# sherholz/mitsuba-path-guiding

Measured on AMD Instinct MI355X. Metric: Mpaths/sec + equal-spp RMSE vs CPU ref, ajar-door scene at 1/2/4/8 GPUs, higher is better.
Workload: dtype f32; 1 GPU; C3 ajar_door 1280x720, guided SD-tree, 5 training iterations (1..16 spp) + 1024 spp render; scene=ajar_door, triangles=58864, width=1280, height=720, spp=1024, parallelism=tile-shard x1, no exchange (one rank)

## Files before the change

### mitsuba-path-guiding_amd/csrc/pg_kernels.h

```cpp
#pragma once
#include <hip/hip_runtime.h>
#include <stdint.h>

#include "pg_layout.h"

struct SceneDev {
    const float4 *nodes;
    const float4 *tris;
    const float4 *wnodes;
    const float4 *wtris;
    const float4 *tshade;
    const uint8_t *tclass;
    const GMat *mats;
    const GEmitter *ems;
    const float4 *emtri;
    const float *emcdf;
    const GEnv *env;
    uint32_t top_nodes;
    uint32_t num_em_boxes;
    float em_absmax;
    float em_box[PG_EMBOX_MAX][6];
    uint32_t num_blockers;
    float absmax;
    uint32_t *blk_counts;
// ... 116 lines not shown
inline uint32_t pg_camera_bound(bool banded, uint32_t npix, uint32_t nlayers) {
    uint32_t b = 0;
    for (uint32_t s = 0; s < 64; ++s) {
        const uint32_t c = pg_camera_count(banded, npix, nlayers, s);
        b = c > b ? c : b;
    }
    return b;
}

void pg_launch_camera(hipStream_t s, const GParams &g, const PathDev &p, const uint32_t *local_pixels,
                      uint32_t pix_begin, uint32_t npix, uint32_t nlayers, uint32_t sample_base, Queue q, bool banded);
void pg_launch_camera_rays(hipStream_t s, const GParams &g, const uint32_t *pixels, const uint32_t *samples, uint32_t n,
                           float *o_tmin, float *d_tmax);
void pg_launch_trace(hipStream_t s, const GParams &g, const SceneDev &sc, const PathDev &p, Queue q, uint32_t max_shard,
                     const Queue *class_queues, bool first_bounce);
void pg_launch_camera_trace(hipStream_t s, const GParams &g, const SceneDev &sc, const PathDev &p,
                            const uint32_t *local_pixels, uint32_t pix_begin, uint32_t npix, uint32_t nlayers,
                            uint32_t sample_base, const Queue *class_queues);
void pg_launch_camera_queue(hipStream_t s, uint32_t npix, uint32_t nlayers, Queue q);
void pg_launch_shade_class(hipStream_t s, int cls, const GParams &g, const SceneDev &sc, const SDDev &sd,
                           const PathDev &p, Queue in, uint32_t max_shard, Queue out, Queue shadow, Queue probe);
void pg_launch_shade_all(hipStream_t s, const GParams &g, const SceneDev &sc, const SDDev &sd, const PathDev &p,
                         const Queue *class_queues, const uint32_t *max_shard, Queue out, Queue shq, Queue probe);
void pg_launch_rays(hipStream_t s, const GParams &g, const SceneDev &sc, const PathDev &p, Queue q, uint32_t max_shard,
                    const Queue *class_queues, Queue shq, uint32_t max_shadow_shard, Queue probe);
void pg_launch_shadow(hipStream_t s, const GParams &g, const SceneDev &sc, const PathDev &p, Queue q, uint32_t max_shard);
void pg_launch_probe(hipStream_t s, const SceneDev &sc, const PathDev &p, Queue probe, uint32_t max_shard,
                     const Queue *class_queues);
void pg_launch_tail(hipStream_t s, const GParams &g, const SceneDev &sc, const SDDev &sd, const PathDev &p, Queue q,
                    uint32_t max_shard, unsigned long long *stats);
void pg_launch_ray_sort(hipStream_t s, Queue q, uint32_t max_shard, uint32_t *sorted_items, uint32_t *hist,
                        uint32_t bins = PG_RAY_SORT_BINS);
void pg_launch_film(hipStream_t s, const GParams &g, const SceneDev &sc, const PathDev &p, const uint32_t *local_pixels,
                    uint32_t pix_begin, uint32_t npix, uint32_t nlayers, float4 *film_rgbw, float4 *film_sumsq,
                    float4 *aov_albedo = nullptr, float4 *aov_normal = nullptr);
struct FilmFilter {
    float radius, scale;
    int32_t border;
// ... 63 lines not shown
```

### mitsuba-path-guiding_amd/csrc/pg_kernels.hip

```cpp
#include <algorithm>
#include <cstdlib>

#include "pg_trace.h"

#ifndef SHADE_LDS_MATS
#define SHADE_LDS_MATS 0
#endif

template <bool LENS>
__global__ __launch_bounds__(256) void k_camera(GParams g, PathDev p, const uint32_t *__restrict__ local_pixels,
                                                uint32_t pix_begin, uint32_t npix, uint32_t nlayers,
                                                uint32_t sample_base, Queue q, bool banded) {
    uint32_t slot = blockIdx.x * blockDim.x + threadIdx.x;
    const uint32_t n = npix * nlayers;
    if (slot < PG_QSHARDS) q.counts[slot] = pg_camera_count(banded, npix, nlayers, slot);
    if (slot >= n) return;
    uint32_t layer = slot / npix, lp = slot - layer * npix;
    uint32_t pix = local_pixels[pix_begin + lp];
    uint32_t sample = sample_base + layer;
    f3 o, wd;
    float tmin, tmax;
    cameraRay<LENS>(g, pix, rngKey(pix, g.seed), sample, o, wd, tmin, tmax);
    stS(pathRayO(p, slot), f4(o, tmin));
    stS(pathRayD(p, slot), f4(wd, tmax));
// ... 122 lines not shown
            }
            cls = hitClass(sc, h, tri, doomed, hr);
            stS(&p.hit[slot], hr);
        }
        classAppend(cls, slot, cqs, s);
    }
}

template <bool ENV, bool CAM>
__global__ __launch_bounds__(TRACE_BLOCK) void k_trace(GParams g, SceneDev sc, PathDev p, Queue q, ClassQueues cqs,
                                                       float4 *first) {
    __shared__ uint32_t stack[LDS_STACK * TRACE_BLOCK];
    traceRows<ENV, CAM>(g, sc, p, q, cqs, first, blockIdx.x, gridDim.x, threadStack(stack, p.stack_ovf));
}

struct CameraChunk {
    const uint32_t *local_pixels;
    uint32_t pix_begin, npix, nlayers, sample_base;
};
template <bool ENV, bool LENS>
__device__ __forceinline__ void cameraRows(const GParams &g, const SceneDev &sc, const PathDev &p, const CameraChunk &cam,
                                           const ClassQueues &cqs, float4 *first, uint32_t bid, uint32_t nblk,
                                           const TStack &stk) {
    const uint32_t s = bid & (PG_QSHARDS - 1);
    const uint32_t n = pg_camera_shard_count(cam.npix * cam.nlayers, s);
    for (uint32_t base = (bid / PG_QSHARDS) * TRACE_BLOCK; base < n; base += nblk / PG_QSHARDS * TRACE_BLOCK) {
        const uint32_t i = base + threadIdx.x;
        int cls = -1;
        uint32_t slot = 0;
        if (i < n) {
            slot = pg_camera_slot(s, i);
            f3 o, wd;
            float tmin, tmax;
            {
                const uint32_t layer = slot / cam.npix, lp = slot - layer * cam.npix;
                const uint32_t pix = cam.local_pixels[cam.pix_begin + lp];
                const uint32_t sample = cam.sample_base + layer;
                cameraRay<LENS>(g, pix, rngKey(pix, g.seed), sample, o, wd, tmin, tmax);
                stS(pathRayD(p, slot), f4(wd, tmax));
                stS(&p.rad[slot], make_float4(0.f, 0.f, 0.f, 0.f));
                stS(pathInfo(p, slot), make_uint4(pix, sample, kCameraWord, 0u));
            }
            const float far = tmax;
            uint32_t tri = 0xFFFFFFFFu;
            float u = 0, v = 0;
            const bool h = traverse<false>(sc.nodes, sc.tris, o, wd, tmin, tmax, tri, u, v, stk);
            float4 hr = make_float4(h ? tmax : 0.0f, __uint_as_float(h ? tri : 0xFFFFFFFFu), u, v);
            if (first) first[slot] = hr;
            if (ENV && !h) {
                const f3 e = envEscapeRadiance(g, sc, p, slot, wd, kCameraWord, far);
                hr = make_float4(e.x, hr.y, e.y, e.z);
            }
            cls = hitClass(sc, h, tri, false, hr);
            stS(&p.hit[slot], hr);
        }
        classAppend(cls, slot, cqs, s);
    }
}
template <bool ENV, bool LENS>
__global__ __launch_bounds__(TRACE_BLOCK) __attribute__((amdgpu_waves_per_eu(LENS ? 4 : ENV ? 5 : 6))) void k_camera_trace(GParams g, SceneDev sc, PathDev p, CameraChunk cam,
                                                              ClassQueues cqs, float4 *first) {
    __shared__ uint32_t stack[LDS_STACK * TRACE_BLOCK];
    cameraRows<ENV, LENS>(g, sc, p, cam, cqs, first, blockIdx.x, gridDim.x, threadStack(stack, p.stack_ovf));
}

__device__ __forceinline__ float shadowTmin(float4 o) {
    return kEpsilon * fmaxf(fmaxf(fabsf(o.x), fabsf(o.y)), fabsf(o.z));
}

template <class T>
__device__ __forceinline__ void waveKeyedAdd(T *base, uint32_t key, T v, bool valid);
__device__ __forceinline__ bool blockerRowCounted(uint32_t row) { return row % PG_BLOCKER_SAMPLE == 0; }
__device__ __forceinline__ void shadowAdd(const PathDev &p, uint32_t slot) {
    float4 c = ldS(&p.sh_c[slot]);
    float4 L = ldS(&p.rad[slot]);
    stS(&p.rad[slot], make_float4(L.x + c.x, L.y + c.y, L.z + c.z, L.w));
    uint32_t vi = __float_as_uint(c.w);
    if (vi != 0xFFFFFFFFu) {
// ... 202 lines not shown
extern "C" int pg_debug_watch_read(float *out, uint32_t max, uint32_t *n) {
    uint32_t w[3];
    if (hipDeviceSynchronize() != hipSuccess) return -1;
    if (hipMemcpyFromSymbol(w, HIP_SYMBOL(pgWatch), sizeof(w)) != hipSuccess) return -1;
    *n = w[2] < PG_WATCH_MAX ? w[2] : PG_WATCH_MAX;
    const uint32_t k = *n < max ? *n : max;
    return hipMemcpyFromSymbol(out, HIP_SYMBOL(pgWatchLog), (size_t)k * PG_WATCH_F * 4) == hipSuccess ? 0 : -1;
}
#define WSET(i, v) (wr[i] = (float)(v))
#define WSET3(i, v) (wr[i] = (v).x, wr[(i) + 1] = (v).y, wr[(i) + 2] = (v).z)
#else
#define WSET(i, v) ((void)0)
#define WSET3(i, v) ((void)0)
#endif

template <int MODEL, bool CAN_GUIDE, bool ENV, bool TEX = false, bool DELTA = false>
__device__ __forceinline__ void shadeOne(const GParams &g, const SceneDev &sc, const SDDev &sd, const PathDev &p,
                                         uint32_t slot, const GMat *mats, bool wantKey, bool &alive, bool &shadow,
                                         bool &probe, uint32_t &rkey, uint32_t &blocked) {
    bool dirtyL = false;
    f3 L = mk1(0.f);
    const bool cull = !PG_WATCH && g.path_cull;
#if PG_WATCH
    float wr[PG_WATCH_F];
    for (int i = 0; i < PG_WATCH_F; ++i) wr[i] = -1.0f;
    bool watched = false;
#endif
    do {
        const uint4 pi = ldS(pathInfo(p, slot));
        const uint32_t pix = pi.x, sample = pi.y;
#if PG_WATCH
        watched = pix == pgWatch[0] && sample == pgWatch[1];
#endif
        const float4 rd4 = ldS(pathRayD(p, slot));
        float4 hv = ldS(&p.hit[slot]);
        uint32_t depth = pi.z & 0xFFFFu, flags = pi.z >> 16, nv = pi.w;
        float4 T4 = depth == 1 ? make_float4(1.f, 1.f, 1.f, 1.f) : ldS(pathThr(p, slot));
        f3 T = xyz(T4);
        bool haveL = depth == 1;
        auto loadL = [&]() {
            if (!haveL) {
                L = xyz(ldS(&p.rad[slot]));
                haveL = true;
            }
        };
        if (PG_WATCH) loadL();
        float eta = T4.w;
        uint32_t tri = __float_as_uint(hv.y);
        if (tri == 0xFFFFFFFFu) break;
        const uint32_t key = rngKey(pix, g.seed);
        f3 rd = xyz(rd4);
        Hit h;
        fetchHit(sc, tri, hv.z, hv.w, rd, h);
        WSET(0, depth);
        WSET(1, __float_as_uint(sc.tshade[(size_t)PG_TRI_SHADE_STRIDE * tri + 2].w));
        WSET3(2, h.p);
        f3 Le = mk1(0.f);
        if (h.emitter >= 0 && dot(h.shN, -rd) > 0) {
            const GEmitter &em = sc.ems[h.emitter];
            Le = mk(em.radiance[0], em.radiance[1], em.radiance[2]);
        }
        if (depth > 1) {
            if (h.emitter >= 0) {
                const float prevPdf = rd4.w;
                float lumPdf = 0.0f;
                if (g.use_nee && !(flags & PF_PREV_DELTA)) {
// ... 194 lines not shown
                             (D - 1 >= (uint32_t)g.rr_depth && rrNext >= fminf(maxc(Tn) * etaN * etaN, 0.95f));
                }
                if (!ENV && doomed && g.doom_probe) {
                    const float po[3] = {h.p.x, h.p.y, h.p.z}, pd[3] = {wo.x, wo.y, wo.z};
                    probe = pg_ray_misses_boxes(sc.em_box, sc.num_em_boxes, sc.em_absmax, po, pd, tmin);
                }
                stS(pathRayO(p, slot), f4(h.p, doomed ? -tmin : tmin));
                stS(pathRayD(p, slot), f4(wo, woPdf));
                if (probe) {
                    stS(&p.hit[slot], make_float4(0.0f, __uint_as_float(0xFFFFFFFFu), 0.0f, 0.0f));
                } else {
                    stS(pathThr(p, slot), f4(Tn, etaN));
                    flags = (flags & ~(PF_EMITTED_QUERY | PF_PREV_DELTA | PF_PREV_FRONT)) |
                        ((bs.type & EDelta) ? PF_PREV_DELTA : 0u) | (doomed ? PF_DOOMED : 0u) |
                        (pg_prev_front(wo.x, wo.y, wo.z, refN.x, refN.y, refN.z) ? PF_PREV_FRONT : 0u);
                    stPinfoZW(pathInfo(p, slot), (depth + 1) | (flags << 16), nv);
                    alive = true;
                    if (wantKey) rkey = rayOrderKey(sd, h.p, wo);
                }
            }
        }
        if (shadow) {
            if (!alive && !probe) stS(pathRayO(p, slot), f4(h.p, 0.0f));
            stS(&p.sh_d[slot], f4(neeD, neeDist * (1 - kShadowEpsilon)));
            stS(&p.sh_c[slot], f4(neeC, __uint_as_float(vtxIndex)));
        }
        if (!alive && nv != pi.w) stPinfoZW(pathInfo(p, slot), pi.z, nv);
    } while (false);
    if (dirtyL) stS(&p.rad[slot], f4(L, 0.0f));
#if PG_WATCH
    if (watched) {
        wr[28] = alive ? 1.0f : 0.0f;
        wr[29] = shadow ? 1.0f : 0.0f;
        const uint32_t k = atomicAdd(&pgWatch[2], 1u);
        if (k < PG_WATCH_MAX)
            for (int i = 0; i < PG_WATCH_F; ++i) pgWatchLog[k * PG_WATCH_F + i] = wr[i];
    }
#endif
}

template <int MODEL, bool CAN_GUIDE, bool ENV, bool TEX = false, bool DELTA = false>
__device__ __forceinline__ void shadeBlock(const GParams &g, const SceneDev &sc, const SDDev &sd, const PathDev &p,
                                           const Queue &in, const Queue &out, const Queue &shq, const Queue &pq,
                                           uint32_t bid) {
    const uint32_t s = bid & (PG_QSHARDS - 1);
    const uint32_t n = in.counts[s];
    {
    const uint32_t base = (bid / PG_QSHARDS) * SHADE_BLOCK;
    if (base >= n) return;
    const uint32_t i = base + threadIdx.x;
    bool alive = false, shadow = false, probe = false;
    uint32_t slot = 0, rkey = 0, blocked = 0;
    if (i < n) slot = in.items[(size_t)s * in.stride + i];
    __shared__ float4 smat[(SHADE_LDS_MATS > 0 ? SHADE_LDS_MATS : 1) * (sizeof(GMat) / 16)];
    const bool ldsMats = SHADE_LDS_MATS > 0 && g.num_materials <= SHADE_LDS_MATS;
    if (ldsMats) {
        const float4 *src = reinterpret_cast<const float4 *>(sc.mats);
        for (uint32_t k = threadIdx.x; k < g.num_materials * (uint32_t)(sizeof(GMat) / 16); k += SHADE_BLOCK) smat[k] = src[k];
        __syncthreads();
    }
    if (i < n)
        shadeOne<MODEL, CAN_GUIDE, ENV, TEX, DELTA>(g, sc, sd, p, slot, ldsMats ? reinterpret_cast<const GMat *>(smat) : sc.mats,
                                        out.keys != nullptr, alive, shadow, probe, rkey, blocked);
    if (out.keys)
        waveAppendKey(alive, slot, (uint16_t)rkey, out.items + (size_t)s * out.stride, out.keys + (size_t)s * out.stride,
                      out.counts + s);
    else
        waveAppend(alive, slot, out.items + (size_t)s * out.stride, out.counts + s);
    waveAppend(shadow, slot, shq.items + (size_t)s * shq.stride, shq.counts + s);
    if (!ENV && sc.num_blockers) {
        const unsigned long long m = __ballot(blocked != 0);
        if (m) {
            if ((threadIdx.x & 63) == 0) atomicAdd(shq.dropped + s, (uint32_t)__popcll(m));
            if (sc.blk_counts && blockerRowCounted(bid / PG_QSHARDS)) {
                waveKeyedAdd<uint32_t>(sc.blk_counts, blocked - 1u, 1u, blocked != 0);
                if ((threadIdx.x & 63) == 0) atomicAdd(sc.blk_total, (uint32_t)__popcll(m));
            }
        }
// ... 2 lines not shown
    }
}

template <int MODEL, bool CAN_GUIDE, bool ENV, bool TEX = false, bool DELTA = false>
__global__ __launch_bounds__(SHADE_BLOCK) void k_shade(GParams g, SceneDev sc, SDDev sd, PathDev p, Queue in,
                                                       Queue out, Queue shq, Queue pq) {
    shadeBlock<MODEL, CAN_GUIDE, ENV, TEX, DELTA>(g, sc, sd, p, in, out, shq, pq, blockIdx.x);
}

struct ShadeRanges {
    uint32_t end[PG_NUM_CLASSES];
};
#ifndef PG_SHADE_WAVES
#define PG_SHADE_WAVES 4
#endif
template <bool TEX, bool DELTA = false>
__global__ __launch_bounds__(SHADE_BLOCK) __attribute__((amdgpu_waves_per_eu(PG_SHADE_WAVES))) void k_shade_all(
    GParams g, SceneDev sc, SDDev sd, PathDev p, ClassQueues in, Queue out, Queue shq, Queue pq, ShadeRanges r) {
    static_assert(PG_NUM_CLASSES == 7, "class ranges");
    const uint32_t b = blockIdx.x;
    if (b < r.end[0]) shadeBlock<PG_BSDF_DIFFUSE, true, false, false, DELTA>(g, sc, sd, p, in.q[0], out, shq, pq, b);
    else if (b < r.end[1]) shadeBlock<PG_BSDF_ROUGHCONDUCTOR, true, false, false, DELTA>(g, sc, sd, p, in.q[1], out, shq, pq, b - r.end[0]);
    else if (b < r.end[2]) shadeBlock<PG_BSDF_ROUGHDIELECTRIC, true, false, false, DELTA>(g, sc, sd, p, in.q[2], out, shq, pq, b - r.end[1]);
    else if (b < r.end[3]) shadeBlock<PG_BSDF_PLASTIC, false, false, false, DELTA>(g, sc, sd, p, in.q[3], out, shq, pq, b - r.end[2]);
    else if (b < r.end[4]) shadeBlock<PG_BSDF_ROUGHPLASTIC, true, false, false, DELTA>(g, sc, sd, p, in.q[4], out, shq, pq, b - r.end[3]);
    else if (!TEX || b < r.end[5]) shadeBlock<-1, false, false, false, DELTA>(g, sc, sd, p, in.q[5], out, shq, pq, b - r.end[4]);
    else if constexpr (TEX)
        shadeBlock<PG_MODELS_TEXTURED, true, false, true, DELTA>(g, sc, sd, p, in.q[6], out, shq, pq, b - r.end[5]);
}

#define RSORT_TILE 4096
template <uint32_t BINS>
__global__ __launch_bounds__(256) void k_rsort_hist(Queue q, uint32_t *hist) {
    __shared__ uint32_t h[BINS];
    const uint32_t s = blockIdx.x & (PG_QSHARDS - 1), tile = blockIdx.x / PG_QSHARDS;
    const uint32_t n = q.counts[s], b0 = tile * RSORT_TILE;
    if (b0 >= n) return;
    for (uint32_t k = threadIdx.x; k < BINS; k += 256) h[k] = 0;
    __syncthreads();
    const uint16_t *keys = q.keys + (size_t)s * q.stride;
    const uint32_t e = min(n, b0 + RSORT_TILE);
    for (uint32_t i = b0 + threadIdx.x; i < e; i += 256) atomicAdd(&h[keys[i]], 1u);
    __syncthreads();
// ... 772 lines not shown
                     const Queue *class_queues, bool first_bounce) {
    if (!max_shard) return;
    ClassQueues cq;
    for (int c = 0; c < PG_CLASS_ROWS; ++c) cq.q[c] = class_queues[c];
    const dim3 grid = shardGrid(max_shard, TRACE_BLOCK, TRACE_MAX_BLOCKS / PG_QSHARDS);
    float4 *first = first_bounce ? p.aov : nullptr;
    if (first_bounce) {
        if (sc.env) hipLaunchKernelGGL((k_trace<true, true>), grid, dim3(TRACE_BLOCK), 0, s, g, sc, p, q, cq, first);
        else hipLaunchKernelGGL((k_trace<false, true>), grid, dim3(TRACE_BLOCK), 0, s, g, sc, p, q, cq, first);
    } else {
        if (sc.env) hipLaunchKernelGGL((k_trace<true, false>), grid, dim3(TRACE_BLOCK), 0, s, g, sc, p, q, cq, first);
        else hipLaunchKernelGGL((k_trace<false, false>), grid, dim3(TRACE_BLOCK), 0, s, g, sc, p, q, cq, first);
    }
}
void pg_launch_camera_trace(hipStream_t s, const GParams &g, const SceneDev &sc, const PathDev &p,
                            const uint32_t *local_pixels, uint32_t pix_begin, uint32_t npix, uint32_t nlayers,
                            uint32_t sample_base, const Queue *class_queues) {
    const uint32_t max_shard = pg_camera_bound(false, npix, nlayers);
    if (!max_shard) return;
    ClassQueues cq;
    for (int c = 0; c < PG_CLASS_ROWS; ++c) cq.q[c] = class_queues[c];
    const dim3 grid = shardGrid(max_shard, TRACE_BLOCK, TRACE_MAX_BLOCKS / PG_QSHARDS), block(TRACE_BLOCK);
    const CameraChunk cam{local_pixels, pix_begin, npix, nlayers, sample_base};
    const bool lens = g.lens_radius > 0;
    if (sc.env) {
        if (lens) hipLaunchKernelGGL((k_camera_trace<true, true>), grid, block, 0, s, g, sc, p, cam, cq, p.aov);
        else hipLaunchKernelGGL((k_camera_trace<true, false>), grid, block, 0, s, g, sc, p, cam, cq, p.aov);
    } else {
        if (lens) hipLaunchKernelGGL((k_camera_trace<false, true>), grid, block, 0, s, g, sc, p, cam, cq, p.aov);
        else hipLaunchKernelGGL((k_camera_trace<false, false>), grid, block, 0, s, g, sc, p, cam, cq, p.aov);
    }
}
void pg_launch_camera_queue(hipStream_t s, uint32_t npix, uint32_t nlayers, Queue q) {
    const uint64_t n = (uint64_t)npix * nlayers;
    if (!n) return;
    hipLaunchKernelGGL(k_camera_queue, dim3(blocks(n, 256)), dim3(256), 0, s, (uint32_t)n, q);
}
template <bool ENV, bool DELTA>
static void launchShade(hipStream_t s, int cls, dim3 grid, const GParams &g, const SceneDev &sc, const SDDev &sd,
                        const PathDev &p, Queue in, Queue out, Queue shq, Queue pq) {
    const dim3 block(SHADE_BLOCK);
    switch (cls) {
        case PG_CLASS_DIFFUSE:
            hipLaunchKernelGGL((k_shade<PG_BSDF_DIFFUSE, true, ENV, false, DELTA>), grid, block, 0, s, g, sc, sd, p, in, out, shq, pq);
            break;
        case PG_CLASS_ROUGHCONDUCTOR:
            hipLaunchKernelGGL((k_shade<PG_BSDF_ROUGHCONDUCTOR, true, ENV, false, DELTA>), grid, block, 0, s, g, sc, sd, p, in, out, shq, pq);
            break;
        case PG_CLASS_ROUGHDIELECTRIC:
            hipLaunchKernelGGL((k_shade<PG_BSDF_ROUGHDIELECTRIC, true, ENV, false, DELTA>), grid, block, 0, s, g, sc, sd, p, in, out, shq, pq);
            break;
// ... 9 lines not shown
        default:
            hipLaunchKernelGGL((k_shade<-1, false, ENV, false, DELTA>), grid, block, 0, s, g, sc, sd, p, in, out, shq, pq);
    }
}
void pg_launch_shade_class(hipStream_t s, int cls, const GParams &g, const SceneDev &sc, const SDDev &sd,
                           const PathDev &p, Queue in, uint32_t max_shard, Queue out, Queue shq, Queue pq) {
    if (!max_shard) return;
    const dim3 grid = shardGrid(max_shard, SHADE_BLOCK, 0xFFFFFFFFu);
    if (sc.delta) {
        if (sc.env) launchShade<true, true>(s, cls, grid, g, sc, sd, p, in, out, shq, pq);
        else launchShade<false, true>(s, cls, grid, g, sc, sd, p, in, out, shq, pq);
    } else if (sc.env) launchShade<true, false>(s, cls, grid, g, sc, sd, p, in, out, shq, pq);
    else launchShade<false, false>(s, cls, grid, g, sc, sd, p, in, out, shq, pq);
}
void pg_launch_shade_all(hipStream_t s, const GParams &g, const SceneDev &sc, const SDDev &sd, const PathDev &p,
                         const Queue *class_queues, const uint32_t *max_shard, Queue out, Queue shq, Queue pq) {
    ClassQueues cq;
    ShadeRanges r;
    uint32_t total = 0;
    for (int c = 0; c < PG_NUM_CLASSES; ++c) {
        cq.q[c] = class_queues[c];
        total += max_shard[c] ? shardGrid(max_shard[c], SHADE_BLOCK, 0xFFFFFFFFu).x : 0;
        r.end[c] = total;
    }
    for (int c = PG_NUM_CLASSES; c < PG_CLASS_ROWS; ++c) cq.q[c] = class_queues[c];
    if (!total) return;
    if (sc.delta) {
        if (sc.mtex) hipLaunchKernelGGL((k_shade_all<true, true>), dim3(total), dim3(SHADE_BLOCK), 0, s, g, sc, sd, p, cq, out, shq, pq, r);
        else hipLaunchKernelGGL((k_shade_all<false, true>), dim3(total), dim3(SHADE_BLOCK), 0, s, g, sc, sd, p, cq, out, shq, pq, r);
    } else if (sc.mtex) hipLaunchKernelGGL(k_shade_all<true>, dim3(total), dim3(SHADE_BLOCK), 0, s, g, sc, sd, p, cq, out, shq, pq, r);
    else hipLaunchKernelGGL(k_shade_all<false>, dim3(total), dim3(SHADE_BLOCK), 0, s, g, sc, sd, p, cq, out, shq, pq, r);
}
static inline bool blockersCounted(const GParams &g, const SceneDev &sc) { return g.record && sc.blk_counts && !sc.env; }
static inline bool probesCounted(const SceneDev &sc) { return sc.prb_counts && !sc.env; }
void pg_launch_rays(hipStream_t s, const GParams &g, const SceneDev &sc, const PathDev &p, Queue q, uint32_t max_shard,
                    const Queue *class_queues, Queue shq, uint32_t max_shadow_shard, Queue pq) {
    ClassQueues cq;
    for (int c = 0; c < PG_CLASS_ROWS; ++c) cq.q[c] = class_queues[c];
    const uint32_t sb = max_shadow_shard ? shardGrid(max_shadow_shard, TRACE_BLOCK, TRACE_MAX_BLOCKS / PG_QSHARDS).x : 0;
    const bool count = blockersCounted(g, sc), pcount = probesCounted(sc);
    const uint32_t pb = (g.doom_probe && !sc.env) ? sb : 0;
    const uint32_t tb =
        max_shard ? shardGrid(max_shard, TRACE_BLOCK, TRACE_MAX_BLOCKS / PG_QSHARDS).x : 0;
    if (sb + tb == 0) return;
    if (tb == 0) {
        if (count) hipLaunchKernelGGL(k_shadow<true>, dim3(sb), dim3(TRACE_BLOCK), 0, s, sc, p, shq);
        else hipLaunchKernelGGL(k_shadow<false>, dim3(sb), dim3(TRACE_BLOCK), 0, s, sc, p, shq);
// ... 217 lines not shown
```

### mitsuba-path-guiding_amd/csrc/pg_pass.cpp

```cpp
#include <algorithm>
#include <chrono>
#include <cmath>
#include <cstdio>
#include <cstdlib>
#include <vector>

#include "pg_chunks.h"
#include "pg_ctx.h"

namespace pgh __attribute__((visibility("hidden"))) {

#ifndef PG_SMALL_PASS
#define PG_SMALL_PASS (1u << 21)
#endif
uint64_t smallPass() {
    static const char *e = std::getenv("PG_SMALL_PASS_PATHS");
    static const uint64_t n = e ? (uint64_t)std::strtoull(e, nullptr, 10) : (uint64_t)PG_SMALL_PASS;
    return n;
}

bool raySortEnabled() {
    static const char *e = std::getenv("PG_RAY_SORT");
    static const bool on = e && std::atoi(e) != 0;
    return on;
// ... 389 lines not shown
    c->stats.vol_vertex_lookups += st[6];
    c->stats.segments += st[0];
    c->stats.shadow_rays += st[1];
    c->stats.density_lookups += st[2];
    if (g.record)
        if (pg_status rs = foldRecordCount(c)) return rs;
    for (EventPair &e : evs) {
        float ms = 0;
        (void)hipEventElapsedTime(&ms, e.a, e.b);
        c->stats.volume_ms += ms;
        c->stats.volume_launches++;
    }
    return PG_OK;
}

EventPair nextEvents(Lane *l, LaunchKind kind) {
    std::vector<EventPair> &pool = l->ev[l->evcur];
    std::vector<uint8_t> &kinds = l->evkind[l->evcur];
    kinds.resize(l->evused[l->evcur] + 1);
    kinds[l->evused[l->evcur]] = (uint8_t)kind;
    if (l->evused[l->evcur] == pool.size()) {
        EventPair e;
        (void)hipEventCreate(&e.a);
        (void)hipEventCreate(&e.b);
        pool.push_back(e);
    }
    return pool[l->evused[l->evcur]++];
}

pg_status collectStats(Ctx *c, Lane &l) {
// ... 100 lines not shown
    }
    const SDDev sd = sdView(c);
    const uint32_t maxBounces = std::min<uint32_t>(g.depth_cap + 2, kMaxBounces);
    const bool evt = c->cfg.kernel_timing != 0;
    const bool fuseRays = !std::getenv("PG_NO_RAYS_FUSION");
    g.path_cull = std::getenv("PG_NO_PATH_CULL") ? 0 : 1;
    g.doom_probe = (g.path_cull && !c->has_env && !std::getenv("PG_NO_DOOM_PROBE")) ? 1 : 0;
    const bool learnProbes = rec && g.doom_probe && !c->prb_stopped && probeListEnabled(c);
    if (learnProbes) {
        sc.prb_counts = c->blk_counts.as<uint32_t>() + c->num_tris + 1;
        sc.prb_total = sc.prb_counts + c->num_tris;
    }
    const bool bands = cameraBands() > 0;
    const bool fuseCamera = !bands && !std::getenv("PG_NO_CAMERA_FUSION");
    const bool fuseShade = !c->has_env && !std::getenv("PG_NO_SHADE_FUSION");
    const std::vector<VChunk> chunks = planChunks(npix, spp, want, sample_offset);
    uint32_t nextChunk = 0, filmNext = 0;
    HIPC(c, hipEventRecord(c->pass_start, c->stream));
    HIPC(c, hipEventRecord(c->film_order, c->stream));
    c->rec_bound = c->rec_host_count;
    hipStream_t laneStreams[PG_MAX_LANES];
    for (int li = 0; li < c->nlanes; ++li) laneStreams[li] = c->lanes[li].stream;
    auto lqueue = [](const Lane &l, uint32_t *items, uint32_t *counts) { return Queue{items, counts, pg_queue_stride(l.P)}; };
    auto traceQueue = [&](const Lane &l, uint32_t b) {
        return lqueue(l, l.sorted ? l.qsorted.as<uint32_t>() : (b & 1) ? l.q1.as<uint32_t>() : l.q0.as<uint32_t>(),
                      l.counters.as<uint32_t>() + (size_t)kBounceWords * b);
    };
    auto classQueues = [&](const Lane &l, uint32_t *cb, Queue *cls) {
        for (int k = 0; k < PG_CLASS_ROWS; ++k)
            cls[k] = lqueue(l, k < PG_NUM_CLASSES ? l.class_q.as<uint32_t>() + (size_t)k * PG_QSHARDS * pg_queue_stride(l.P)
                                                 : nullptr,
                            cb + kClassCounts + k * PG_QSHARDS);
    };
    auto launchTrace = [&](Lane &l, const Queue *shq, const Queue *pq) -> pg_status {
        uint32_t *cb = l.counters.as<uint32_t>() + (size_t)kBounceWords * l.b;
        Queue cls[PG_CLASS_ROWS];
        classQueues(l, cb, cls);
        EventPair et{};
        if (evt) et = nextEvents(&l, shq ? KT_RAYS : KT_TRACE);
        if (evt) HIPC(c, hipEventRecord(et.a, l.stream));
        const Queue tq = traceQueue(l, l.b);
        if (shq) pg_launch_rays(l.stream, g, sc, pathView(&l), tq, l.bound, cls, *shq, l.bound, *pq);
        else if (l.b == 0 && fuseCamera)
            pg_launch_camera_trace(l.stream, g, sc, pathView(&l), c->d_band_pixels.as<uint32_t>(), l.pb, l.np, l.nl,
                                   l.sample_base, cls);
        else pg_launch_trace(l.stream, g, sc, pathView(&l), tq, l.bound, cls, l.b == 0);
        if (evt) HIPC(c, hipEventRecord(et.b, l.stream));
        HIPC(c, hipMemcpyAsync(l.h_counts + (size_t)kBounceWords * l.b + kClassCounts, cb + kClassCounts,
                               PG_CLASS_ROWS * PG_QSHARDS * 4, hipMemcpyDeviceToHost, l.stream));
        HIPC(c, hipEventRecord(l.ready, l.stream));
        return PG_OK;
    };
    auto startChunk = [&](Lane &l) -> pg_status {
        l.active = false;
        if (nextChunk >= chunks.size()) return PG_OK;
        if (c->cancel.load()) return fail(c, PG_ERR_CANCELLED, "cancelled");
        const VChunk &ch = chunks[nextChunk];
        l.pb = ch.pb, l.np = ch.np, l.nl = ch.nl, l.sample_base = ch.sample_base;
        l.b = 0;
        l.sorted = false;
        l.bound = pg_camera_bound(pg_camera_banded(bands, l.np), l.np, l.nl);
// ... 48 lines not shown
                m = std::max(m, v);
                shardLive[sh] += v;
                nlive += v;
            }
            if (k < PG_NUM_CLASSES) clsMax[k] = m;
        }
        {
            uint64_t t = 0;
            for (int w = 0; w < PG_CLASS_ROWS * PG_QSHARDS; ++w) t += hc[w];
            l.used_cur.push_back(t);
        }
        ++l.b;
        const uint32_t tailMax = c->cfg.tail_paths < 0 ? 0u : c->cfg.tail_paths > 0 ? (uint32_t)c->cfg.tail_paths : tailPaths();
        const bool tail = nlive > 0 && nlive <= tailMax && l.b < maxBounces;
        if (tail) {
            if (l.b == 1 && fuseCamera) pg_launch_camera_queue(l.stream, l.np, l.nl, traceQueue(l, 0));
            pg_launch_tail(l.stream, g, sc, sd, pathView(&l), traceQueue(l, l.b - 1), l.bound,
                           l.tail_stats.as<unsigned long long>());
            c->stats.tail_launches += 1;
        }
        if (nlive == 0 || tail || l.b >= maxBounces) {
            l.traced = true;
            for (int k = 0; k < c->nlanes; ++k) {
                Lane &o = c->lanes[k];
                if (!(o.active && o.traced && o.chunk == filmNext)) continue;
                ++filmNext;
                if (pg_status st = finishChunk(o)) return st;
                k = -1;
            }
            return PG_OK;
        }
        Queue cls[PG_CLASS_ROWS];
        classQueues(l, cb, cls);
        const PathDev pv = pathView(&l);
        Queue next = lqueue(l, (l.b & 1) ? l.q1.as<uint32_t>() : l.q0.as<uint32_t>(), cb + kBounceWords);
        Queue shq = lqueue(l, l.qs.as<uint32_t>(), cb + kShadowCounts);
        shq.dropped = cb + kDropCounts;
        Queue pq = lqueue(l, l.qp.as<uint32_t>(), cb + kProbeCounts);
        pq.dropped = cb + kResolvedCounts;
        const uint32_t nextBound = *std::max_element(shardLive, shardLive + PG_QSHARDS);
        const bool sortNext = raySortEnabled() && nextBound >= kRaySortMinShard;
        if (sortNext) next.keys = l.qkey.as<uint16_t>();
        EventPair es{}, ew{};
        if (evt) es = nextEvents(&l, KT_SHADE);
        if (evt) HIPC(c, hipEventRecord(es.a, l.stream));
        if (fuseShade) {
            pg_launch_shade_all(l.stream, g, sc, sd, pv, cls, clsMax, next, shq, pq);
            c->stats.shade_launches += 1;
        } else {
            for (int k = 0; k < PG_NUM_CLASSES; ++k) {
                pg_launch_shade_class(l.stream, k, g, sc, sd, pv, cls[k], clsMax[k], next, shq, pq);
                c->stats.shade_launches += clsMax[k] ? 1 : 0;
            }
        }
        if (evt) HIPC(c, hipEventRecord(es.b, l.stream));
        l.bound = nextBound;
        if (sortNext)
            pg_launch_ray_sort(l.stream, next, l.bound, l.qsorted.as<uint32_t>(), l.rsort_hist.as<uint32_t>());
        l.sorted = sortNext;
        if (fuseRays) return launchTrace(l, &shq, &pq);
        if (evt) ew = nextEvents(&l, KT_SHADOW);
        if (evt) HIPC(c, hipEventRecord(ew.a, l.stream));
// ... 41 lines not shown
        if (l.stream) (void)hipStreamSynchronize(l.stream);
        l.npending = false;
        if (l.span.a) (void)hipEventDestroy(l.span.a);
        if (l.span.b) (void)hipEventDestroy(l.span.b);
        l.span = EventPair{};
        l.active = l.waved = false;
    }
    if (c->stream) (void)hipStreamSynchronize(c->stream);
}

}

using namespace pgh;

extern "C" {

pg_status pg_render_pass(void *ctx, uint32_t spp, uint32_t sample_offset, int32_t record) {
    Ctx *c = (Ctx *)ctx;
    if (!c) return fail(nullptr, PG_ERR_INVALID, "pg_render_pass: null context");
    if (!c->has_scene) return fail(c, PG_ERR_STATE, "pg_render_pass: no scene uploaded");
    if (c->cancel.load()) return fail(c, PG_ERR_CANCELLED, "cancelled");
    HIPC(c, hipSetDevice(c->cfg.device));
    c->rendered = true;
    const pg_status s = renderPass(c, spp, sample_offset, record);
    if (s) drainLanes(c);
    return s;
}

pg_status pg_render_time(void *ctx, double seconds, uint32_t spp_per_progression, uint32_t sample_offset,
                         uint32_t max_spp, uint32_t *spp_done) {
// ... 27 lines not shown
```

Measured before the change: 959.0 Mpaths/s.

## Recompute first-bounce camera ray state in shading instead of storing it

Adds a lean camera-trace variant that skips writing ray direction and path info for primary rays. The fused shade kernel then regenerates pixel, sample and camera direction for the first bounce from the chunk description. A separate camera-state kernel rebuilds the stored state when the tail path needs it. This cuts global memory writes and reads per primary path in exchange for recomputing camera rays and more template variants. It also adds atomic debug counters on the host.

```diff
diff --git a/mitsuba-path-guiding_amd/csrc/pg_kernels.h b/mitsuba-path-guiding_amd/csrc/pg_kernels.h
--- a/mitsuba-path-guiding_amd/csrc/pg_kernels.h
+++ b/mitsuba-path-guiding_amd/csrc/pg_kernels.h
@@ -154,14 +154,20 @@
                            float *o_tmin, float *d_tmax);
 void pg_launch_trace(hipStream_t s, const GParams &g, const SceneDev &sc, const PathDev &p, Queue q, uint32_t max_shard,
                      const Queue *class_queues, bool first_bounce);
+struct CameraChunk {
+    const uint32_t *local_pixels;
+    uint32_t pix_begin, npix, nlayers, sample_base;
+};
 void pg_launch_camera_trace(hipStream_t s, const GParams &g, const SceneDev &sc, const PathDev &p,
-                            const uint32_t *local_pixels, uint32_t pix_begin, uint32_t npix, uint32_t nlayers,
-                            uint32_t sample_base, const Queue *class_queues);
+                            const CameraChunk &cam, const Queue *class_queues, bool lean = false);
 void pg_launch_camera_queue(hipStream_t s, uint32_t npix, uint32_t nlayers, Queue q);
+void pg_launch_camera_state(hipStream_t s, const GParams &g, const PathDev &p, const CameraChunk &cam, Queue q);
 void pg_launch_shade_class(hipStream_t s, int cls, const GParams &g, const SceneDev &sc, const SDDev &sd,
                            const PathDev &p, Queue in, uint32_t max_shard, Queue out, Queue shadow, Queue probe);
 void pg_launch_shade_all(hipStream_t s, const GParams &g, const SceneDev &sc, const SDDev &sd, const PathDev &p,
-                         const Queue *class_queues, const uint32_t *max_shard, Queue out, Queue shq, Queue probe);
+                         const Queue *class_queues, const uint32_t *max_shard, Queue out, Queue shq, Queue probe,
+                         const CameraChunk *first = nullptr);
+bool pg_first_recompute_ok(const SceneDev &sc);
 void pg_launch_rays(hipStream_t s, const GParams &g, const SceneDev &sc, const PathDev &p, Queue q, uint32_t max_shard,
                     const Queue *class_queues, Queue shq, uint32_t max_shadow_shard, Queue probe);
 void pg_launch_shadow(hipStream_t s, const GParams &g, const SceneDev &sc, const PathDev &p, Queue q, uint32_t max_shard);
diff --git a/mitsuba-path-guiding_amd/csrc/pg_kernels.hip b/mitsuba-path-guiding_amd/csrc/pg_kernels.hip
--- a/mitsuba-path-guiding_amd/csrc/pg_kernels.hip
+++ b/mitsuba-path-guiding_amd/csrc/pg_kernels.hip
@@ -1,5 +1,6 @@
 #include <algorithm>
 #include <cstdlib>
+#include <type_traits>
 
 #include "pg_trace.h"
 
@@ -160,11 +161,12 @@
     traceRows<ENV, CAM>(g, sc, p, q, cqs, first, blockIdx.x, gridDim.x, threadStack(stack, p.stack_ovf));
 }
 
-struct CameraChunk {
-    const uint32_t *local_pixels;
-    uint32_t pix_begin, npix, nlayers, sample_base;
-};
-template <bool ENV, bool LENS>
+__device__ __forceinline__ void cameraSample(const CameraChunk &cam, uint32_t slot, uint32_t &pix, uint32_t &sample) {
+    const uint32_t layer = slot / cam.npix, lp = slot - layer * cam.npix;
+    pix = cam.local_pixels[cam.pix_begin + lp];
+    sample = cam.sample_base + layer;
+}
+template <bool ENV, bool LENS, bool LEAN>
 __device__ __forceinline__ void cameraRows(const GParams &g, const SceneDev &sc, const PathDev &p, const CameraChunk &cam,
                                            const ClassQueues &cqs, float4 *first, uint32_t bid, uint32_t nblk,
                                            const TStack &stk) {
@@ -179,13 +181,12 @@
             f3 o, wd;
             float tmin, tmax;
             {
-                const uint32_t layer = slot / cam.npix, lp = slot - layer * cam.npix;
-                const uint32_t pix = cam.local_pixels[cam.pix_begin + lp];
-                const uint32_t sample = cam.sample_base + layer;
+                uint32_t pix, sample;
+                cameraSample(cam, slot, pix, sample);
                 cameraRay<LENS>(g, pix, rngKey(pix, g.seed), sample, o, wd, tmin, tmax);
-                stS(pathRayD(p, slot), f4(wd, tmax));
+                if (!LEAN) stS(pathRayD(p, slot), f4(wd, tmax));
                 stS(&p.rad[slot], make_float4(0.f, 0.f, 0.f, 0.f));
-                stS(pathInfo(p, slot), make_uint4(pix, sample, kCameraWord, 0u));
+                if (!LEAN || g.record) stS(pathInfo(p, slot), make_uint4(pix, sample, kCameraWord, 0u));
             }
             const float far = tmax;
             uint32_t tri = 0xFFFFFFFFu;
@@ -203,11 +204,27 @@
         classAppend(cls, slot, cqs, s);
     }
 }
-template <bool ENV, bool LENS>
+template <bool ENV, bool LENS, bool LEAN = false>
 __global__ __launch_bounds__(TRACE_BLOCK) __attribute__((amdgpu_waves_per_eu(LENS ? 4 : ENV ? 5 : 6))) void k_camera_trace(GParams g, SceneDev sc, PathDev p, CameraChunk cam,
                                                               ClassQueues cqs, float4 *first) {
+    static_assert(!(ENV && LEAN), "the environment emitter's launches read the camera rows");
     __shared__ uint32_t stack[LDS_STACK * TRACE_BLOCK];
-    cameraRows<ENV, LENS>(g, sc, p, cam, cqs, first, blockIdx.x, gridDim.x, threadStack(stack, p.stack_ovf));
+    cameraRows<ENV, LENS, LEAN>(g, sc, p, cam, cqs, first, blockIdx.x, gridDim.x, threadStack(stack, p.stack_ovf));
+}
+template <bool LENS>
+__global__ __launch_bounds__(256) void k_camera_state(GParams g, PathDev p, CameraChunk cam, Queue q) {
+    const uint32_t slot = blockIdx.x * blockDim.x + threadIdx.x;
+    const uint32_t n = cam.npix * cam.nlayers;
+    if (slot < PG_QSHARDS) q.counts[slot] = pg_camera_shard_count(n, slot);
+    if (slot >= n) return;
+    q.items[pg_camera_shard(slot) * q.stride + pg_camera_entry(slot)] = slot;
+    uint32_t pix, sample;
+    cameraSample(cam, slot, pix, sample);
+    f3 o, wd;
+    float tmin, tmax;
+    cameraRay<LENS>(g, pix, rngKey(pix, g.seed), sample, o, wd, tmin, tmax);
+    stS(pathRayD(p, slot), f4(wd, tmax));
+    stS(pathInfo(p, slot), make_uint4(pix, sample, kCameraWord, 0u));
 }
 
 __device__ __forceinline__ float shadowTmin(float4 o) {
@@ -440,10 +457,12 @@
 #define WSET3(i, v) ((void)0)
 #endif
 
-template <int MODEL, bool CAN_GUIDE, bool ENV, bool TEX = false, bool DELTA = false>
+constexpr int kFirstPinhole = 1, kFirstLens = 2;
+template <int MODEL, bool CAN_GUIDE, bool ENV, bool TEX = false, bool DELTA = false, int FIRST = 0>
 __device__ __forceinline__ void shadeOne(const GParams &g, const SceneDev &sc, const SDDev &sd, const PathDev &p,
                                          uint32_t slot, const GMat *mats, bool wantKey, bool &alive, bool &shadow,
-                                         bool &probe, uint32_t &rkey, uint32_t &blocked) {
+                                         bool &probe, uint32_t &rkey, uint32_t &blocked,
+                                         const CameraChunk *cam = nullptr) {
     bool dirtyL = false;
     f3 L = mk1(0.f);
     const bool cull = !PG_WATCH && g.path_cull;
@@ -453,12 +472,20 @@
     bool watched = false;
 #endif
     do {
-        const uint4 pi = ldS(pathInfo(p, slot));
+        uint4 pi;
+        if constexpr (FIRST) {
+            cameraSample(*cam, slot, pi.x, pi.y);
+            pi.z = kCameraWord;
+            pi.w = 0u;
+        } else {
+            pi = ldS(pathInfo(p, slot));
+        }
         const uint32_t pix = pi.x, sample = pi.y;
 #if PG_WATCH
         watched = pix == pgWatch[0] && sample == pgWatch[1];
 #endif
-        const float4 rd4 = ldS(pathRayD(p, slot));
+        float4 rd4 = make_float4(0.f, 0.f, 0.f, 0.f);
+        if constexpr (!FIRST) rd4 = ldS(pathRayD(p, slot));
         float4 hv = ldS(&p.hit[slot]);
         uint32_t depth = pi.z & 0xFFFFu, flags = pi.z >> 16, nv = pi.w;
         float4 T4 = depth == 1 ? make_float4(1.f, 1.f, 1.f, 1.f) : ldS(pathThr(p, slot));
@@ -476,6 +503,11 @@
         if (tri == 0xFFFFFFFFu) break;
         const uint32_t key = rngKey(pix, g.seed);
         f3 rd = xyz(rd4);
+        if constexpr (FIRST) {
+            f3 co;
+            float ctmin, ctmax;
+            cameraRay<FIRST == kFirstLens>(g, pix, key, sample, co, rd, ctmin, ctmax);
+        }
         Hit h;
         fetchHit(sc, tri, hv.z, hv.w, rd, h);
         WSET(0, depth);
@@ -700,7 +732,8 @@
                     flags = (flags & ~(PF_EMITTED_QUERY | PF_PREV_DELTA | PF_PREV_FRONT)) |
                         ((bs.type & EDelta) ? PF_PREV_DELTA : 0u) | (doomed ? PF_DOOMED : 0u) |
                         (pg_prev_front(wo.x, wo.y, wo.z, refN.x, refN.y, refN.z) ? PF_PREV_FRONT : 0u);
-                    stPinfoZW(pathInfo(p, slot), (depth + 1) | (flags << 16), nv);
+                    if constexpr (FIRST) stS(pathInfo(p, slot), make_uint4(pix, sample, (depth + 1) | (flags << 16), nv));
+                    else stPinfoZW(pathInfo(p, slot), (depth + 1) | (flags << 16), nv);
                     alive = true;
                     if (wantKey) rkey = rayOrderKey(sd, h.p, wo);
                 }
@@ -711,7 +744,10 @@
             stS(&p.sh_d[slot], f4(neeD, neeDist * (1 - kShadowEpsilon)));
             stS(&p.sh_c[slot], f4(neeC, __uint_as_float(vtxIndex)));
         }
-        if (!alive && nv != pi.w) stPinfoZW(pathInfo(p, slot), pi.z, nv);
+        if (!alive && nv != pi.w) {
+            if constexpr (FIRST) stS(pathInfo(p, slot), make_uint4(pix, sample, pi.z, nv));
+            else stPinfoZW(pathInfo(p, slot), pi.z, nv);
+        }
     } while (false);
     if (dirtyL) stS(&p.rad[slot], f4(L, 0.0f));
 #if PG_WATCH
@@ -725,10 +761,10 @@
 #endif
 }
 
-template <int MODEL, bool CAN_GUIDE, bool ENV, bool TEX = false, bool DELTA = false>
+template <int MODEL, bool CAN_GUIDE, bool ENV, bool TEX = false, bool DELTA = false, int FIRST = 0>
 __device__ __forceinline__ void shadeBlock(const GParams &g, const SceneDev &sc, const SDDev &sd, const PathDev &p,
                                            const Queue &in, const Queue &out, const Queue &shq, const Queue &pq,
-                                           uint32_t bid) {
+                                           uint32_t bid, const CameraChunk *cam = nullptr) {
     const uint32_t s = bid & (PG_QSHARDS - 1);
     const uint32_t n = in.counts[s];
     {
@@ -746,8 +782,8 @@
         __syncthreads();
     }
     if (i < n)
-        shadeOne<MODEL, CAN_GUIDE, ENV, TEX, DELTA>(g, sc, sd, p, slot, ldsMats ? reinterpret_cast<const GMat *>(smat) : sc.mats,
-                                        out.keys != nullptr, alive, shadow, probe, rkey, blocked);
+        shadeOne<MODEL, CAN_GUIDE, ENV, TEX, DELTA, FIRST>(g, sc, sd, p, slot, ldsMats ? reinterpret_cast<const GMat *>(smat) : sc.mats,
+                                        out.keys != nullptr, alive, shadow, probe, rkey, blocked, cam);
     if (out.keys)
         waveAppendKey(alive, slot, (uint16_t)rkey, out.items + (size_t)s * out.stride, out.keys + (size_t)s * out.stride,
                       out.counts + s);
@@ -780,19 +816,23 @@
 #ifndef PG_SHADE_WAVES
 #define PG_SHADE_WAVES 4
 #endif
-template <bool TEX, bool DELTA = false>
+struct NoCamera {};
+template <bool TEX, bool DELTA = false, int FIRST = 0>
 __global__ __launch_bounds__(SHADE_BLOCK) __attribute__((amdgpu_waves_per_eu(PG_SHADE_WAVES))) void k_shade_all(
-    GParams g, SceneDev sc, SDDev sd, PathDev p, ClassQueues in, Queue out, Queue shq, Queue pq, ShadeRanges r) {
+    GParams g, SceneDev sc, SDDev sd, PathDev p, ClassQueues in, Queue out, Queue shq, Queue pq, ShadeRanges r,
+    std::conditional_t<FIRST != 0, CameraChunk, NoCamera> first) {
     static_assert(PG_NUM_CLASSES == 7, "class ranges");
+    const CameraChunk *cam = nullptr;
+    if constexpr (FIRST != 0) cam = &first;
     const uint32_t b = blockIdx.x;
-    if (b < r.end[0]) shadeBlock<PG_BSDF_DIFFUSE, true, false, false, DELTA>(g, sc, sd, p, in.q[0], out, shq, pq, b);
-    else if (b < r.end[1]) shadeBlock<PG_BSDF_ROUGHCONDUCTOR, true, false, false, DELTA>(g, sc, sd, p, in.q[1], out, shq, pq, b - r.end[0]);
-    else if (b < r.end[2]) shadeBlock<PG_BSDF_ROUGHDIELECTRIC, true, false, false, DELTA>(g, sc, sd, p, in.q[2], out, shq, pq, b - r.end[1]);
-    else if (b < r.end[3]) shadeBlock<PG_BSDF_PLASTIC, false, false, false, DELTA>(g, sc, sd, p, in.q[3], out, shq, pq, b - r.end[2]);
-    else if (b < r.end[4]) shadeBlock<PG_BSDF_ROUGHPLASTIC, true, false, false, DELTA>(g, sc, sd, p, in.q[4], out, shq, pq, b - r.end[3]);
-    else if (!TEX || b < r.end[5]) shadeBlock<-1, false, false, false, DELTA>(g, sc, sd, p, in.q[5], out, shq, pq, b - r.end[4]);
+    if (b < r.end[0]) shadeBlock<PG_BSDF_DIFFUSE, true, false, false, DELTA, FIRST>(g, sc, sd, p, in.q[0], out, shq, pq, b, cam);
+    else if (b < r.end[1]) shadeBlock<PG_BSDF_ROUGHCONDUCTOR, true, false, false, DELTA, FIRST>(g, sc, sd, p, in.q[1], out, shq, pq, b - r.end[0], cam);
+    else if (b < r.end[2]) shadeBlock<PG_BSDF_ROUGHDIELECTRIC, true, false, false, DELTA, FIRST>(g, sc, sd, p, in.q[2], out, shq, pq, b - r.end[1], cam);
+    else if (b < r.end[3]) shadeBlock<PG_BSDF_PLASTIC, false, false, false, DELTA, FIRST>(g, sc, sd, p, in.q[3], out, shq, pq, b - r.end[2], cam);
+    else if (b < r.end[4]) shadeBlock<PG_BSDF_ROUGHPLASTIC, true, false, false, DELTA, FIRST>(g, sc, sd, p, in.q[4], out, shq, pq, b - r.end[3], cam);
+    else if (!TEX || b < r.end[5]) shadeBlock<-1, false, false, false, DELTA, FIRST>(g, sc, sd, p, in.q[5], out, shq, pq, b - r.end[4], cam);
     else if constexpr (TEX)
-        shadeBlock<PG_MODELS_TEXTURED, true, false, true, DELTA>(g, sc, sd, p, in.q[6], out, shq, pq, b - r.end[5]);
+        shadeBlock<PG_MODELS_TEXTURED, true, false, true, DELTA, FIRST>(g, sc, sd, p, in.q[6], out, shq, pq, b - r.end[5], cam);
 }
 
 #define RSORT_TILE 4096
@@ -1595,16 +1635,17 @@
     }
 }
 void pg_launch_camera_trace(hipStream_t s, const GParams &g, const SceneDev &sc, const PathDev &p,
-                            const uint32_t *local_pixels, uint32_t pix_begin, uint32_t npix, uint32_t nlayers,
-                            uint32_t sample_base, const Queue *class_queues) {
-    const uint32_t max_shard = pg_camera_bound(false, npix, nlayers);
+                            const CameraChunk &cam, const Queue *class_queues, bool lean) {
+    const uint32_t max_shard = pg_camera_bound(false, cam.npix, cam.nlayers);
     if (!max_shard) return;
     ClassQueues cq;
     for (int c = 0; c < PG_CLASS_ROWS; ++c) cq.q[c] = class_queues[c];
     const dim3 grid = shardGrid(max_shard, TRACE_BLOCK, TRACE_MAX_BLOCKS / PG_QSHARDS), block(TRACE_BLOCK);
-    const CameraChunk cam{local_pixels, pix_begin, npix, nlayers, sample_base};
     const bool lens = g.lens_radius > 0;
-    if (sc.env) {
+    if (lean && !sc.env) {
+        if (lens) hipLaunchKernelGGL((k_camera_trace<false, true, true>), grid, block, 0, s, g, sc, p, cam, cq, p.aov);
+        else hipLaunchKernelGGL((k_camera_trace<false, false, true>), grid, block, 0, s, g, sc, p, cam, cq, p.aov);
+    } else if (sc.env) {
         if (lens) hipLaunchKernelGGL((k_camera_trace<true, true>), grid, block, 0, s, g, sc, p, cam, cq, p.aov);
         else hipLaunchKernelGGL((k_camera_trace<true, false>), grid, block, 0, s, g, sc, p, cam, cq, p.aov);
     } else {
@@ -1616,6 +1657,12 @@
     const uint64_t n = (uint64_t)npix * nlayers;
     if (!n) return;
     hipLaunchKernelGGL(k_camera_queue, dim3(blocks(n, 256)), dim3(256), 0, s, (uint32_t)n, q);
+}
+void pg_launch_camera_state(hipStream_t s, const GParams &g, const PathDev &p, const CameraChunk &cam, Queue q) {
+    const uint64_t n = (uint64_t)cam.npix * cam.nlayers;
+    if (!n) return;
+    if (g.lens_radius > 0) hipLaunchKernelGGL(k_camera_state<true>, dim3(blocks(n, 256)), dim3(256), 0, s, g, p, cam, q);
+    else hipLaunchKernelGGL(k_camera_state<false>, dim3(blocks(n, 256)), dim3(256), 0, s, g, p, cam, q);
 }
 template <bool ENV, bool DELTA>
 static void launchShade(hipStream_t s, int cls, dim3 grid, const GParams &g, const SceneDev &sc, const SDDev &sd,
@@ -1655,7 +1702,8 @@
     else launchShade<false, false>(s, cls, grid, g, sc, sd, p, in, out, shq, pq);
 }
 void pg_launch_shade_all(hipStream_t s, const GParams &g, const SceneDev &sc, const SDDev &sd, const PathDev &p,
-                         const Queue *class_queues, const uint32_t *max_shard, Queue out, Queue shq, Queue pq) {
+                         const Queue *class_queues, const uint32_t *max_shard, Queue out, Queue shq, Queue pq,
+                         const CameraChunk *first) {
     ClassQueues cq;
     ShadeRanges r;
     uint32_t total = 0;
@@ -1666,12 +1714,23 @@
     }
     for (int c = PG_NUM_CLASSES; c < PG_CLASS_ROWS; ++c) cq.q[c] = class_queues[c];
     if (!total) return;
+    const dim3 grid(total), block(SHADE_BLOCK);
+    if (first) {
+        if (g.lens_radius > 0) {
+            if (sc.mtex) hipLaunchKernelGGL((k_shade_all<true, false, kFirstLens>), grid, block, 0, s, g, sc, sd, p, cq, out, shq, pq, r, *first);
+            else hipLaunchKernelGGL((k_shade_all<false, false, kFirstLens>), grid, block, 0, s, g, sc, sd, p, cq, out, shq, pq, r, *first);
+        } else if (sc.mtex) hipLaunchKernelGGL((k_shade_all<true, false, kFirstPinhole>), grid, block, 0, s, g, sc, sd, p, cq, out, shq, pq, r, *first);
+        else hipLaunchKernelGGL((k_shade_all<false, false, kFirstPinhole>), grid, block, 0, s, g, sc, sd, p, cq, out, shq, pq, r, *first);
+        return;
+    }
+    const NoCamera none;
     if (sc.delta) {
-        if (sc.mtex) hipLaunchKernelGGL((k_shade_all<true, true>), dim3(total), dim3(SHADE_BLOCK), 0, s, g, sc, sd, p, cq, out, shq, pq, r);
-        else hipLaunchKernelGGL((k_shade_all<false, true>), dim3(total), dim3(SHADE_BLOCK), 0, s, g, sc, sd, p, cq, out, shq, pq, r);
-    } else if (sc.mtex) hipLaunchKernelGGL(k_shade_all<true>, dim3(total), dim3(SHADE_BLOCK), 0, s, g, sc, sd, p, cq, out, shq, pq, r);
-    else hipLaunchKernelGGL(k_shade_all<false>, dim3(total), dim3(SHADE_BLOCK), 0, s, g, sc, sd, p, cq, out, shq, pq, r);
-}
+        if (sc.mtex) hipLaunchKernelGGL((k_shade_all<true, true>), grid, block, 0, s, g, sc, sd, p, cq, out, shq, pq, r, none);
+        else hipLaunchKernelGGL((k_shade_all<false, true>), grid, block, 0, s, g, sc, sd, p, cq, out, shq, pq, r, none);
+    } else if (sc.mtex) hipLaunchKernelGGL(k_shade_all<true>, grid, block, 0, s, g, sc, sd, p, cq, out, shq, pq, r, none);
+    else hipLaunchKernelGGL(k_shade_all<false>, grid, block, 0, s, g, sc, sd, p, cq, out, shq, pq, r, none);
+}
+bool pg_first_recompute_ok(const SceneDev &sc) { return !sc.env && !sc.delta; }
 static inline bool blockersCounted(const GParams &g, const SceneDev &sc) { return g.record && sc.blk_counts && !sc.env; }
 static inline bool probesCounted(const SceneDev &sc) { return sc.prb_counts && !sc.env; }
 void pg_launch_rays(hipStream_t s, const GParams &g, const SceneDev &sc, const PathDev &p, Queue q, uint32_t max_shard,
diff --git a/mitsuba-path-guiding_amd/csrc/pg_pass.cpp b/mitsuba-path-guiding_amd/csrc/pg_pass.cpp
--- a/mitsuba-path-guiding_amd/csrc/pg_pass.cpp
+++ b/mitsuba-path-guiding_amd/csrc/pg_pass.cpp
@@ -1,4 +1,5 @@
 #include <algorithm>
+#include <atomic>
 #include <chrono>
 #include <cmath>
 #include <cstdio>
@@ -427,6 +428,8 @@
     return PG_OK;
 }
 
+std::atomic<unsigned long long> firstVertexCounts[3];
+
 EventPair nextEvents(Lane *l, LaunchKind kind) {
     std::vector<EventPair> &pool = l->ev[l->evcur];
     std::vector<uint8_t> &kinds = l->evkind[l->evcur];
@@ -557,6 +560,7 @@
     const bool bands = cameraBands() > 0;
     const bool fuseCamera = !bands && !std::getenv("PG_NO_CAMERA_FUSION");
     const bool fuseShade = !c->has_env && !std::getenv("PG_NO_SHADE_FUSION");
+    const bool leanFirst = fuseCamera && fuseShade && pg_first_recompute_ok(sc) && !std::getenv("PG_NO_FIRST_RECOMPUTE");
     const std::vector<VChunk> chunks = planChunks(npix, spp, want, sample_offset);
     uint32_t nextChunk = 0, filmNext = 0;
     HIPC(c, hipEventRecord(c->pass_start, c->stream));
@@ -565,6 +569,7 @@
     hipStream_t laneStreams[PG_MAX_LANES];
     for (int li = 0; li < c->nlanes; ++li) laneStreams[li] = c->lanes[li].stream;
     auto lqueue = [](const Lane &l, uint32_t *items, uint32_t *counts) { return Queue{items, counts, pg_queue_stride(l.P)}; };
+    auto cameraChunk = [&](const Lane &l) { return CameraChunk{c->d_band_pixels.as<uint32_t>(), l.pb, l.np, l.nl, l.sample_base}; };
     auto traceQueue = [&](const Lane &l, uint32_t b) {
         return lqueue(l, l.sorted ? l.qsorted.as<uint32_t>() : (b & 1) ? l.q1.as<uint32_t>() : l.q0.as<uint32_t>(),
                       l.counters.as<uint32_t>() + (size_t)kBounceWords * b);
@@ -584,10 +589,10 @@
         if (evt) HIPC(c, hipEventRecord(et.a, l.stream));
         const Queue tq = traceQueue(l, l.b);
         if (shq) pg_launch_rays(l.stream, g, sc, pathView(&l), tq, l.bound, cls, *shq, l.bound, *pq);
-        else if (l.b == 0 && fuseCamera)
-            pg_launch_camera_trace(l.stream, g, sc, pathView(&l), c->d_band_pixels.as<uint32_t>(), l.pb, l.np, l.nl,
-                                   l.sample_base, cls);
-        else pg_launch_trace(l.stream, g, sc, pathView(&l), tq, l.bound, cls, l.b == 0);
+        else if (l.b == 0 && fuseCamera) {
+            pg_launch_camera_trace(l.stream, g, sc, pathView(&l), cameraChunk(l), cls, leanFirst);
+            if (leanFirst) firstVertexCounts[0]++;
+        } else pg_launch_trace(l.stream, g, sc, pathView(&l), tq, l.bound, cls, l.b == 0);
         if (evt) HIPC(c, hipEventRecord(et.b, l.stream));
         HIPC(c, hipMemcpyAsync(l.h_counts + (size_t)kBounceWords * l.b + kClassCounts, cb + kClassCounts,
                                PG_CLASS_ROWS * PG_QSHARDS * 4, hipMemcpyDeviceToHost, l.stream));
@@ -666,7 +671,10 @@
         const uint32_t tailMax = c->cfg.tail_paths < 0 ? 0u : c->cfg.tail_paths > 0 ? (uint32_t)c->cfg.tail_paths : tailPaths();
         const bool tail = nlive > 0 && nlive <= tailMax && l.b < maxBounces;
         if (tail) {
-            if (l.b == 1 && fuseCamera) pg_launch_camera_queue(l.stream, l.np, l.nl, traceQueue(l, 0));
+            if (l.b == 1 && leanFirst) {
+                pg_launch_camera_state(l.stream, g, pathView(&l), cameraChunk(l), traceQueue(l, 0));
+                firstVertexCounts[2]++;
+            } else if (l.b == 1 && fuseCamera) pg_launch_camera_queue(l.stream, l.np, l.nl, traceQueue(l, 0));
             pg_launch_tail(l.stream, g, sc, sd, pathView(&l), traceQueue(l, l.b - 1), l.bound,
                            l.tail_stats.as<unsigned long long>());
             c->stats.tail_launches += 1;
@@ -697,7 +705,10 @@
         if (evt) es = nextEvents(&l, KT_SHADE);
         if (evt) HIPC(c, hipEventRecord(es.a, l.stream));
         if (fuseShade) {
-            pg_launch_shade_all(l.stream, g, sc, sd, pv, cls, clsMax, next, shq, pq);
+            const CameraChunk cam = cameraChunk(l);
+            const bool first = l.b == 1 && leanFirst;
+            pg_launch_shade_all(l.stream, g, sc, sd, pv, cls, clsMax, next, shq, pq, first ? &cam : nullptr);
+            if (first) firstVertexCounts[1]++;
             c->stats.shade_launches += 1;
         } else {
             for (int k = 0; k < PG_NUM_CLASSES; ++k) {
@@ -769,6 +780,13 @@
 using namespace pgh;
 
 extern "C" {
+
+void pg_debug_first_vertex(unsigned long long *out, int reset) {
+    for (int i = 0; i < 3; ++i) {
+        out[i] = firstVertexCounts[i].load();
+        if (reset) firstVertexCounts[i].store(0);
+    }
+}
 
 pg_status pg_render_pass(void *ctx, uint32_t spp, uint32_t sample_offset, int32_t record) {
     Ctx *c = (Ctx *)ctx;
```

Result: no change. 958.5 Mpaths/s (-0.1%).
